# Arief-AK/OpenCL-Development-Real-time-Image-Processing

Hardware: AMD Instinct MI355X
Metric: Mpixels/s (Gaussian 5x5, 4K RGBA) (higher is better)
Workload: dtype u8 in/out, f32 accumulate

## Files before the change

### include/mi355_imgfilter.h

```cpp
#ifndef MI355_IMGFILTER_H
#define MI355_IMGFILTER_H

#include <stddef.h>
#include <stdint.h>

#ifdef __cplusplus
extern "C" {
#endif

#define MI355_OK 0
#define MI355_ERR_BAD_ARG (-1)
#define MI355_ERR_HIP (-2)
#define MI355_ERR_NO_DEVICE (-3)
#define MI355_ERR_UNSUPPORTED (-4)
#define MI355_ERR_NOMEM (-5)

#define MI355_MAX_GAUSS_K 63

#define MI355_GAUSS_FAST 0
#define MI355_GAUSS_EXACT 1

typedef struct mi355_ctx mi355_ctx;

int mi355_device_count(int* count);
// ... 15 lines not shown

#define MI355_INPUT_RGBA 0
#define MI355_INPUT_BGR 1
int mi355_ctx_set_input_format(mi355_ctx* ctx, int format);
int mi355_bgr_to_rgba8_dev(mi355_ctx* ctx, const void* d_bgr, void* d_rgba, int w, int h, int nframes);

int mi355_gauss_weights(int k, float sigma, float* out_k2);
int mi355_ctx_set_gauss_weights(mi355_ctx* ctx, int k, float sigma, const float* w_k2);

int mi355_gray_rgba8(mi355_ctx* ctx, const uint8_t* rgba, uint8_t* out_rgba, int w, int h,
                     uint64_t prof_ns[6]);
int mi355_gray1_rgba8(mi355_ctx* ctx, const uint8_t* rgba, uint8_t* out_gray, int w, int h,
                      uint64_t prof_ns[6]);
int mi355_gauss_rgba8(mi355_ctx* ctx, const uint8_t* rgba, uint8_t* out_rgba, int w, int h, int k,
                      float sigma, uint64_t prof_ns[6]);
int mi355_sobel_rgba8(mi355_ctx* ctx, const uint8_t* rgba, uint8_t* out_gray, int w, int h,
                      uint64_t prof_ns[6]);
int mi355_pipeline_rgba8(mi355_ctx* ctx, const uint8_t* rgba, uint8_t* out_gray, int w, int h, int k,
                         float sigma, uint64_t prof_ns[6]);

int mi355_image2d_rgba8(mi355_ctx* ctx, int filter, const uint8_t* rgba, uint8_t* out, int w, int h, int k,
                        float sigma, uint64_t prof_ns[6]);
int mi355_gauss_weights_image2d(int k, float sigma, float* out_k2);

#define MI355_FILTER_GRAY 0
#define MI355_FILTER_GRAY1 1
#define MI355_FILTER_GAUSS 2
#define MI355_FILTER_SOBEL 3
#define MI355_FILTER_PIPELINE 4
#define MI355_FILTER_GAUSS_GRAY8 5
#define MI355_FILTER_SOBEL_GRAY8 6
#define MI355_FILTER_PIPELINE_GRAY8 7
#define MI355_MAX_MEDIAN_K 7
#define MI355_FILTER_MEDIAN 16
#define MI355_FILTER_MEDIAN_GRAY8 17
#define MI355_MAX_MORPH_K 17
#define MI355_FILTER_ERODE 24
#define MI355_FILTER_DILATE 25
#define MI355_FILTER_OPEN 26
#define MI355_FILTER_CLOSE 27
#define MI355_FILTER_ERODE_GRAY8 28
#define MI355_FILTER_DILATE_GRAY8 29
#define MI355_FILTER_OPEN_GRAY8 30
#define MI355_FILTER_CLOSE_GRAY8 31
#define MI355_FILTER_EQUALIZE_GRAY8 40
#define MI355_FILTER_OTSU_GRAY8 41
#define MI355_MAX_BOX_K 63
#define MI355_FILTER_BOX 48
#define MI355_FILTER_BOX_GRAY8 49
int mi355_filter_batched(mi355_ctx* ctx, int filter, const uint8_t* rgba, uint8_t* out, int w, int h,
                         int nframes, int k, float sigma, uint64_t prof_ns[6]);
int mi355_filter_out_bpp(int filter);
int mi355_filter_in_bpp(int filter);

int mi355_filter_stream(mi355_ctx* ctx, int filter, const uint8_t* rgba, uint8_t* out, int w, int h,
                        int nframes, int chunk_frames, int k, float sigma, double* elapsed_ms);
int mi355_host_alloc(mi355_ctx* ctx, size_t nbytes, void** h_ptr);
int mi355_host_free(mi355_ctx* ctx, void* h_ptr);

int mi355_gray_rgba8_dev(mi355_ctx* ctx, const void* d_in, void* d_out, int w, int h, int nframes);
int mi355_gray1_rgba8_dev(mi355_ctx* ctx, const void* d_in, void* d_out, int w, int h, int nframes);
int mi355_gauss_rgba8_dev(mi355_ctx* ctx, const void* d_in, void* d_out, int w, int h, int nframes,
                          int k, float sigma);
int mi355_sobel_rgba8_dev(mi355_ctx* ctx, const void* d_in, void* d_out, int w, int h, int nframes);
int mi355_pipeline_rgba8_dev(mi355_ctx* ctx, const void* d_in, void* d_out, int w, int h, int nframes,
                             int k, float sigma);
int mi355_filter_dev(mi355_ctx* ctx, int filter, const void* d_in, void* d_out, int w, int h,
                     int nframes, int k, float sigma);
int mi355_hist_gray8_dev(mi355_ctx* ctx, const void* d_in, uint32_t* d_hist, int w, int h, int nframes);
int mi355_otsu_thresholds_gray8_dev(mi355_ctx* ctx, const void* d_in, int32_t* d_thresh, int w, int h, int nframes);

#define MI355_INTERP_NEAREST 0
#define MI355_INTERP_LINEAR 1
#define MI355_INTERP_AREA 3
#define MI355_MAX_AREA_FACTOR 16
int mi355_resize_check(int bpp, int src_w, int src_h, int dst_w, int dst_h, int nframes, int interp);
int mi355_resize_dev(mi355_ctx* ctx, const void* d_in, void* d_out, int bpp, int src_w, int src_h,
                     int dst_w, int dst_h, int nframes, int interp);
int mi355_resize_batched(mi355_ctx* ctx, const uint8_t* in, uint8_t* out, int bpp, int src_w, int src_h,
                         int dst_w, int dst_h, int nframes, int interp, uint64_t prof_ns[6]);

#define MI355_WARP_INVERSE_MAP 16
#define MI355_BORDER_CONSTANT 0
#define MI355_BORDER_REPLICATE 1
#define MI355_MAX_WARP_SIZE 32766
int mi355_rotation_matrix(double cx, double cy, double angle_deg, double scale, double m[6]);
int mi355_warp_affine_matrix(const double m[6], int flags, double inv[6]);
int mi355_warp_affine_check(int bpp, int src_w, int src_h, int dst_w, int dst_h, int nframes, const double m[6],
                            int flags, int border_mode);
int mi355_warp_affine_dev(mi355_ctx* ctx, const void* d_in, void* d_out, int bpp, int src_w, int src_h, int dst_w,
                          int dst_h, int nframes, const double m[6], int flags, int border_mode,
                          uint32_t border_value);
int mi355_warp_affine_batched(mi355_ctx* ctx, const uint8_t* in, uint8_t* out, int bpp, int src_w, int src_h,
                              int dst_w, int dst_h, int nframes, const double m[6], int flags, int border_mode,
                              uint32_t border_value, uint64_t prof_ns[6]);

#define MI355_MAP_FIXED 0
#define MI355_MAP_FLOAT 1
int mi355_remap_check(int bpp, int src_w, int src_h, int dst_w, int dst_h, int nframes, int map_kind, int interp,
                      int border_mode);
int mi355_remap_dev(mi355_ctx* ctx, const void* d_in, void* d_out, int bpp, int src_w, int src_h, int dst_w, int dst_h,
                    int nframes, const void* d_map1, const void* d_map2, int map_kind, int interp, int border_mode,
                    uint32_t border_value);
int mi355_remap_batched(mi355_ctx* ctx, const uint8_t* in, uint8_t* out, int bpp, int src_w, int src_h, int dst_w,
                        int dst_h, int nframes, const void* map1, const void* map2, int map_kind, int interp,
                        int border_mode, uint32_t border_value, uint64_t prof_ns[6]);
// ... 91 lines not shown
```

### opencl-development-real-time-image-processing_amd/__init__.py

```python
from .imgfilter import (
    ADAPTIVE_BINARY,
    ADAPTIVE_BINARY_INV,
    BORDER_CONSTANT,
    BORDER_REPLICATE,
    FILTER_BOX,
    FILTER_BOX_GRAY8,
    FILTER_CLOSE,
    FILTER_CLOSE_GRAY8,
    FILTER_DILATE,
    FILTER_DILATE_GRAY8,
    FILTER_ERODE,
    FILTER_ERODE_GRAY8,
    FILTER_EQUALIZE_GRAY8,
    FILTER_GAUSS,
    FILTER_GAUSS_GRAY8,
    FILTER_GRAY,
    FILTER_GRAY1,
    FILTER_MEDIAN,
    FILTER_MEDIAN_GRAY8,
    FILTER_OPEN,
    FILTER_OPEN_GRAY8,
    FILTER_OTSU_GRAY8,
    FILTER_PIPELINE,
    FILTER_PIPELINE_GRAY8,
    FILTER_SOBEL,
    FILTER_SOBEL_GRAY8,
    IN_BPP,
    OUT_BPP,
    GAUSS_EXACT,
    GAUSS_FAST,
    IMPL_AUTO,
    IMPL_MFMA,
    INPUT_BGR,
    INTERP_AREA,
    INTERP_LINEAR,
    INTERP_NEAREST,
    INPUT_RGBA,
    IMPL_TILE,
    IMPL_VALU,
    MAP_FIXED,
    MAP_FLOAT,
    MAX_AREA_FACTOR,
    MAX_BOX_K,
    MAX_CLAHE_TILES,
    MAX_MEDIAN_K,
    MAX_MORPH_K,
    MAX_WARP_SIZE,
    WARP_INVERSE_MAP,
    YUV_BT601,
    YUV_BT601_FULL,
    YUV_BT709,
    YUV_I420,
    YUV_NV12,
    YUV_NV21,
    YUV_UYVY,
    YUV_YUY2,
    YUV_YV12,
    Context,
    Group,
    Mi355Error,
    adaptive_threshold_check,
    build_library,
    clahe_check,
    declared_symbols,
    gauss_weights,
    gauss_weights_image2d,
    group_shard,
    library_path,
    load_library,
    perspective_matrix,
    remap_check,
    resize_check,
    rotation_matrix,
    warp_affine_check,
    warp_affine_matrix,
    warp_perspective_check,
    yuv_check,
    yuv_frame_bytes,
)
```

### opencl-development-real-time-image-processing_amd/csrc/capi.hip

```cpp
#include <hip/hip_runtime.h>

#include <cmath>
#include <cstdio>
#include <cstdlib>
#include <cstring>
#include <ctime>
#include <new>
#include <vector>

#include "../../include/mi355_imgfilter.h"
#include "kernels.hpp"

using namespace mi355;

namespace {

struct CoefEntry {
    int k;
    uint32_t sigma_bits;
    GaussCoef coef;
    float* d_buf;
    std::vector<float> h_tab;
    uint64_t last_use;
    bool installed;
// ... 853 lines not shown
}

MI355_API int mi355_gauss_weights_image2d(int k, float sigma, float* out_k2)
{
    if (!out_k2 || !valid_k(k) || !valid_sigma(sigma))
        return MI355_ERR_BAD_ARG;
    gen_weights_image2d(k, sigma, out_k2);
    return MI355_OK;
}

MI355_API int mi355_image2d_rgba8(mi355_ctx* ctx, int filter, const uint8_t* rgba, uint8_t* out, int w, int h, int k,
                                  float sigma, uint64_t prof_ns[6])
{
    if (!ctx || !rgba || !out || !valid_sizes(w, h, 1) ||
        (filter != MI355_FILTER_GRAY && filter != MI355_FILTER_GAUSS && filter != MI355_FILTER_SOBEL))
        return MI355_ERR_BAD_ARG;
    const bool gauss = filter == MI355_FILTER_GAUSS;
    if (gauss && (!valid_k(k) || !valid_sigma(sigma)))
        return MI355_ERR_BAD_ARG;
    HIP_TRY(ctx, hipSetDevice(ctx->device));
    const size_t npx = (size_t)w * h, in_bytes = npx * 4, out_bytes = npx * (gauss ? 4 : 1);
    int rc = ensure(ctx, ctx->d_in, in_bytes);
    if (rc == MI355_OK)
        rc = ensure(ctx, ctx->d_out, out_bytes);
    if (rc != MI355_OK)
        return rc;
    if (gauss) {
        if (!ctx->d_img_table)
            HIP_TRY(ctx, hipMalloc((void**)&ctx->d_img_table, sizeof(float) * MI355_MAX_GAUSS_K * MI355_MAX_GAUSS_K));
        std::vector<float> table((size_t)k * k);
        gen_weights_image2d(k, sigma, table.data());
        HIP_TRY(ctx, hipStreamSynchronize(ctx->stream));
        HIP_TRY(ctx, hipMemcpy(ctx->d_img_table, table.data(), sizeof(float) * table.size(), hipMemcpyHostToDevice));
    }
    return timed_roundtrip(ctx, ctx->d_in.p, rgba, in_bytes, out, out_bytes, prof_ns, [&] {
        HIP_TRY(ctx, launch_image2d(ctx->stream, filter, static_cast<const uint8_t*>(ctx->d_in.p),
                                    static_cast<uint8_t*>(ctx->d_out.p), w, h, 1, k, ctx->d_img_table));
        return MI355_OK;
    });
}

MI355_API int mi355_ctx_set_gauss_weights(mi355_ctx* ctx, int k, float sigma, const float* w_k2)
{
    if (!ctx || !w_k2 || !valid_k(k) || !valid_sigma(sigma))
        return MI355_ERR_BAD_ARG;
    for (int i = 0; i < k * k; i++)
        if (!std::isfinite(w_k2[i]))
            return MI355_ERR_BAD_ARG;
    HIP_TRY(ctx, hipSetDevice(ctx->device));
    HIP_TRY(ctx, hipStreamSynchronize(ctx->stream));
    return install_coef(ctx, k, sigma, w_k2, true, nullptr);
}

MI355_API int mi355_filter_out_bpp(int filter)
{
    const FilterInfo* f = filter_info(filter);
    return f ? f->out_bpp : MI355_ERR_BAD_ARG;
}

MI355_API int mi355_filter_in_bpp(int filter)
{
    const FilterInfo* f = filter_info(filter);
    return f ? f->in_bpp : MI355_ERR_BAD_ARG;
}

MI355_API int mi355_gray_rgba8(mi355_ctx* ctx, const uint8_t* rgba, uint8_t* out, int w, int h,
                               uint64_t prof_ns[6])
{
    return run_host(ctx, MI355_FILTER_GRAY, rgba, out, w, h, 1, 0, 0.0f, prof_ns);
}

MI355_API int mi355_gray1_rgba8(mi355_ctx* ctx, const uint8_t* rgba, uint8_t* out, int w, int h,
                                uint64_t prof_ns[6])
{
    return run_host(ctx, MI355_FILTER_GRAY1, rgba, out, w, h, 1, 0, 0.0f, prof_ns);
}

MI355_API int mi355_gauss_rgba8(mi355_ctx* ctx, const uint8_t* rgba, uint8_t* out, int w, int h, int k,
                                float sigma, uint64_t prof_ns[6])
{
    return run_host(ctx, MI355_FILTER_GAUSS, rgba, out, w, h, 1, k, sigma, prof_ns);
}

MI355_API int mi355_sobel_rgba8(mi355_ctx* ctx, const uint8_t* rgba, uint8_t* out, int w, int h,
                                uint64_t prof_ns[6])
{
    return run_host(ctx, MI355_FILTER_SOBEL, rgba, out, w, h, 1, 0, 0.0f, prof_ns);
}

MI355_API int mi355_pipeline_rgba8(mi355_ctx* ctx, const uint8_t* rgba, uint8_t* out, int w, int h,
                                   int k, float sigma, uint64_t prof_ns[6])
{
    return run_host(ctx, MI355_FILTER_PIPELINE, rgba, out, w, h, 1, k, sigma, prof_ns);
}

MI355_API int mi355_filter_batched(mi355_ctx* ctx, int filter, const uint8_t* rgba, uint8_t* out, int w,
                                   int h, int nframes, int k, float sigma, uint64_t prof_ns[6])
{
    return run_host(ctx, filter, rgba, out, w, h, nframes, k, sigma, prof_ns);
}

MI355_API int mi355_host_alloc(mi355_ctx* ctx, size_t nbytes, void** h_ptr)
{
    if (!ctx || !h_ptr || nbytes == 0)
        return MI355_ERR_BAD_ARG;
    HIP_TRY(ctx, hipSetDevice(ctx->device));
// ... 948 lines not shown
```

### opencl-development-real-time-image-processing_amd/csrc/gauss_slide.hip

```cpp
#include <cmath>
#include <cstdlib>
#include <type_traits>

#include "common.hpp"
#include "kernels.hpp"
#include "slide_common.hpp"

namespace mi355 {

namespace {

constexpr uint32_t kRowStoreNowhere = 0x80000000u;
__device__ __forceinline__ void gstore_row_nt(global_ptr<uint8_t> rowp, uint32_t row_bytes, uint32_t off, u32x4 v)
{
    const auto rsrc = __builtin_amdgcn_make_buffer_rsrc((void*)rowp, (short)0, (int)row_bytes, 0x00020000);
    __builtin_amdgcn_raw_buffer_store_b128(v, rsrc, (int)off, 0, 2 );
}

constexpr uint32_t kSlideLdsForFiveWaves = 160u * 1024u / 5u - 1024u;
template <typename... KArgs, typename... Args>
hipError_t launch_slide_lds(void (*kernel)(KArgs...), const BandPlan& plan, uint32_t lds_bytes, hipStream_t stream,
                            Args... args)
{
    hipLaunchKernelGGL(kernel, dim3(plan.nblocks_a + plan.nblocks_b), dim3(kSlideWavesPerBlock * 64), lds_bytes, stream,
// ... 414 lines not shown
    L.g = slide_geom<4>(it.strip, lanes_out, lane, w, 16u, 16u);
    L.y0 = it.y0;
    L.nout = it.nout;
    L.h = h;
    L.w = w;
    L.row_bytes = (size_t)w * 4;
    L.fin = uniform_ptr(in + it.frame * L.row_bytes * h);
    L.fout = uniform_ptr(out + it.frame * L.row_bytes * h);
    L.edge = RaggedEdge{false, false, false, false};
    if constexpr (RAGGED) {
        if (w >= 4)
            L.g.in_off = ragged_edge_setup(L.g.q_lane, L.g.q_load, w, &L.edge);
    }
#pragma unroll
    for (int j = 0; j < 4; j++)
        L.px_off[j] = (uint32_t)clampi(L.g.x_lane + j, 0, w - 1) * 4u;

    float wv[K];
#pragma unroll
    for (int j = 0; j < K; j++) {
        wv[j] = wts.w[j];
        asm volatile("" : "+v"(wv[j]));
    }

    const bool up = (it.band & 1) != 0;
    u32x4 q3[K];
    auto run = [&](auto amode, bool preloaded) -> int {
        constexpr int AMODE = decltype(amode)::value;
        constexpr int NCH = AMODE == 0 ? 4 : 3;
        if constexpr (R <= 3) {
            if (up)
                return gauss_slide_band<R, CLAMP, NCH, RAGGED, true, AMODE, LOCKSTEP>(L, wv, alpha_hi, alpha_tab, q3, preloaded);
        }
        return gauss_slide_band<R, CLAMP, NCH, RAGGED, false, AMODE, LOCKSTEP>(L, wv, alpha_hi, alpha_tab, q3, preloaded);
    };
    auto three_channels = [&]() -> int {
        int code = run(std::integral_constant<int, 1>{}, false);
        if (code == kBandAbortUniform || code == kBandAbortUniformFirst)
            code = run(std::integral_constant<int, 2>{}, code == kBandAbortUniformFirst);
        return code;
    };
    if constexpr (MODE == 0) {
        if (three_channels() != kBandDone)
            run(std::integral_constant<int, 0>{}, false);
    } else if constexpr (MODE == 3) {
        const int code = three_channels();
        if (lane == 0)
            flags[it.work] = code == kBandDone ? 0u : 1u;
    } else {
        run(std::integral_constant<int, 0>{}, false);
    }
}

template <int R>
bool slide_plan(int w, int h, int nframes, bool ragged, StripPlan* sp, BandPlan* plan)
{
    constexpr int K = 2 * R + 1;
    *sp = make_strip_plan(w);
    if (K == 5) {
        const bool big = (size_t)sp->nstrips * ((h + 23) / 24) * nframes >= 2800;
        const int rows = (big && !ragged) ? 15 : 24;
        return make_band_plan(h, sp->nstrips, nframes, 4, rows, rows, rows, 0.0, 12, plan);
    }
    return (K == 3)   ? make_band_plan(h, sp->nstrips, nframes, 5, 12, 12, 12, 0.0, 6, plan)
                      : make_band_plan(h, sp->nstrips, nframes, 3, 96, 270, 40, 0.1, 4 * R + 4, plan);
}

template <int R>
hipError_t launch_r(hipStream_t stream, const uint8_t* d_in, uint8_t* d_out, int w, int h, int nframes,
                    const GaussCoef& coef, uint32_t* d_flags)
{
    constexpr int K = 2 * R + 1;
    constexpr bool kSplit = R >= 3;
    StripPlan sp;
    BandPlan plan;
    const bool ragged = rows_ragged(w, d_in, 16, d_out, 16) || (size_t)w * 4 > kRowStoreNowhere;
    if (!slide_plan<R>(w, h, nframes, ragged, &sp, &plan) || (kSplit && !d_flags))
        return hipErrorInvalidValue;
    const int nstrips = sp.nstrips, lanes_out = sp.lanes_out;
    Weights<K> wts;
    for (int j = 0; j < K; j++)
        wts.w[j] = coef.h_w1d[j];
    double wsum = 0.0;
    for (int j = 0; j < K; j++)
        wsum += (double)coef.h_w1d[j];
    if (!coef.d_alpha_tab)
        return hipErrorInvalidValue;
    const uint32_t alpha_hi = coef.h_alpha_tab[255];
    const uint32_t* alpha_tab = coef.d_alpha_tab;
    const bool lockstep =
        R <= 2 && !ragged && nstrips % kSlideWavesPerBlock == 0 && plan.nwork_b == 0 && plan.nwork_a >= 8192u;
    const uint32_t lds_bytes = (R == 1 && !ragged) ? kSlideLdsForFiveWaves : 0u;
    auto launch = [&](auto kernel) {
        return launch_slide_lds(kernel, plan, lds_bytes, stream, d_in, d_out, w, h, nstrips, lanes_out, plan, wts, alpha_hi,
                                alpha_tab, d_flags);
    };
    return dispatch_bool(gauss_upper_clamp(wsum), [&](auto CL) {
        return dispatch_bool(ragged, [&](auto RG) {
            if constexpr (kSplit) {
                const hipError_t e = launch(gauss_slide_kernel<R, CL.value, RG.value, 3, false>);
                return e != hipSuccess ? e : launch(gauss_slide_kernel<R, CL.value, RG.value, 4, false>);
            } else if constexpr (RG.value) {
                return launch(gauss_slide_kernel<R, CL.value, true, 0, false>);
            } else {
                return dispatch_bool(
                    lockstep, [&](auto LS) { return launch(gauss_slide_kernel<R, CL.value, false, 0, LS.value>); });
            }
        });
    });
}

}

bool gauss_slide_supported(const uint8_t* d_in, const uint8_t* d_out, int w, int h, int k)
{
    (void)h;
    (void)w;
    if (k != 3 && k != 5 && k != 7 && k != 9)
        return false;
    return aligned_to(d_in, 4) && aligned_to(d_out, 4);
}

size_t gauss_slide_flag_items(int w, int h, int nframes, int k)
{
    StripPlan sp;
    BandPlan plan;
    const hipError_t e = dispatch_int(k, std::integer_sequence<int, 7, 9>{}, [&](auto K) {
        return slide_plan<K.value / 2>(w, h, nframes, false, &sp, &plan) ? hipSuccess : hipErrorInvalidValue;
    });
    return e == hipSuccess ? (size_t)plan.nwork_a + plan.nwork_b : 0;
}

hipError_t launch_gauss_slide(hipStream_t stream, const uint8_t* d_in, uint8_t* d_out, int w, int h,
                              int nframes, const GaussCoef& coef, uint32_t* d_flags)
{
    return dispatch_int(coef.k, std::integer_sequence<int, 3, 5, 7, 9>{}, [&](auto K) {
        return launch_r<K.value / 2>(stream, d_in, d_out, w, h, nframes, coef, d_flags);
    });
}

}
```

### opencl-development-real-time-image-processing_amd/csrc/kernels.hpp

```cpp
#pragma once
#include <hip/hip_runtime.h>
#include <stdint.h>

namespace mi355 {

struct GaussCoef {
    int k;
    const float* d_w2d;
    const float* d_w1d;
    float h_w1d[64];
    const float* h_w2d;
    bool separable;
    const uint32_t* d_alpha_tab;
    uint32_t h_alpha_tab[256];
    const uint32_t* d_alpha_cpu;
    uint32_t h_alpha_cpu[256];
};

uint32_t gauss_const_alpha(const float* w1d, int k, uint32_t a);

hipError_t launch_gray(hipStream_t stream, const uint8_t* d_in, uint8_t* d_out, int w, int h,
                       int nframes, bool one_channel);

size_t gauss_flag_items(const uint8_t* d_in, const uint8_t* d_out, int w, int h, int nframes, const GaussCoef& coef,
                        bool exact, int impl);
hipError_t launch_gauss(hipStream_t stream, const uint8_t* d_in, uint8_t* d_out, int w, int h,
                        int nframes, const GaussCoef& coef, bool exact, int impl, uint32_t* d_flags);

hipError_t launch_gauss_tile(hipStream_t stream, const uint8_t* d_in, uint8_t* d_out, int w, int h,
                             int nframes, const GaussCoef& coef, bool exact);

bool gauss_slide_supported(const uint8_t* d_in, const uint8_t* d_out, int w, int h, int k);
size_t gauss_slide_flag_items(int w, int h, int nframes, int k);
hipError_t launch_gauss_slide(hipStream_t stream, const uint8_t* d_in, uint8_t* d_out, int w, int h,
                              int nframes, const GaussCoef& coef, uint32_t* d_flags);

bool gauss_wide_supported(const uint8_t* d_in, const uint8_t* d_out, int w, int h, int k);
size_t gauss_wide_flag_items(int w, int h, int nframes, int k);
hipError_t launch_gauss_wide(hipStream_t stream, const uint8_t* d_in, uint8_t* d_out, int w, int h, int nframes,
                             const GaussCoef& coef, uint32_t* d_flags);

bool gauss_exact_supported(const uint8_t* d_in, const uint8_t* d_out, int w, int h, const GaussCoef& coef);
hipError_t launch_gauss_exact(hipStream_t stream, const uint8_t* d_in, uint8_t* d_out, int w, int h, int nframes,
                              const GaussCoef& coef);

bool gauss_mfma_reg_supported(const uint8_t* d_in, const uint8_t* d_out, int w, int h, const GaussCoef& coef);
hipError_t launch_gauss_mfma_reg(hipStream_t stream, const uint8_t* d_in, uint8_t* d_out, int w, int h, int nframes,
                                 const GaussCoef& coef);

hipError_t launch_sobel(hipStream_t stream, const uint8_t* d_in, uint8_t* d_out, int w, int h,
                        int nframes, int impl);
bool sobel_slide_supported(const uint8_t* d_in, const uint8_t* d_out, int w, int h);
hipError_t launch_sobel_slide(hipStream_t stream, const uint8_t* d_in, uint8_t* d_out, int w, int h, int nframes);

hipError_t launch_pipeline(hipStream_t stream, const uint8_t* d_in, uint8_t* d_out, int w, int h,
                           int nframes, const GaussCoef& coef, bool exact, int impl);
bool pipe_slide_supported(const uint8_t* d_in, const uint8_t* d_out, int w, int h, const GaussCoef& coef, int px);
hipError_t launch_pipe_slide(hipStream_t stream, const uint8_t* d_in, uint8_t* d_out, int w, int h, int nframes,
                             const GaussCoef& coef, int px);

hipError_t launch_gauss_gray8(hipStream_t stream, const uint8_t* d_in, uint8_t* d_out, int w, int h, int nframes,
                              const GaussCoef& coef, bool exact, int impl);
hipError_t launch_sobel_gray8(hipStream_t stream, const uint8_t* d_in, uint8_t* d_out, int w, int h, int nframes);
hipError_t launch_pipeline_gray8(hipStream_t stream, const uint8_t* d_in, uint8_t* d_out, int w, int h, int nframes,
                                 const GaussCoef& coef, int impl);

hipError_t launch_median(hipStream_t stream, const uint8_t* d_in, uint8_t* d_out, int w, int h, int nframes, int k,
                         bool gray8, int impl);

hipError_t launch_morph(hipStream_t stream, const uint8_t* d_in, uint8_t* d_out, int w, int h, int nframes, int k,
                        int op, bool gray8);

hipError_t launch_hist(hipStream_t stream, const uint8_t* d_in, uint32_t* d_hist, int w, int h, int nframes);
hipError_t launch_hist_table(hipStream_t stream, const uint32_t* d_hist, uint8_t* d_lut, int32_t* d_thresh, int w,
                             int h, int nframes, bool otsu);
hipError_t launch_lut_apply(hipStream_t stream, const uint8_t* d_in, uint8_t* d_out, const uint8_t* d_lut, int w, int h,
                            int nframes);

constexpr int kClaheMaxTiles = 16;
struct ClaheGeom {
    int w, h, tiles_x, tiles_y;
    int tw, th;
    int cl;
    float lut_scale, inv_tw, inv_th;
};
hipError_t launch_clahe_hist(hipStream_t stream, const uint8_t* d_in, uint32_t* d_hist, const ClaheGeom& g, int nframes);
hipError_t launch_clahe_table(hipStream_t stream, const uint32_t* d_hist, uint8_t* d_luts, const ClaheGeom& g,
                              int nframes);
// ... 69 lines not shown
```

### opencl-development-real-time-image-processing_amd/imgfilter.py

```python
import ctypes
import os
import re
import subprocess

import numpy as np

_HERE = os.path.dirname(os.path.abspath(__file__))
_ROOT = os.path.dirname(_HERE)
_LIB = os.path.join(_HERE, "lib", "libmi355_imgfilter.so")
_HEADER = os.path.join(_ROOT, "include", "mi355_imgfilter.h")

FILTER_GRAY, FILTER_GRAY1, FILTER_GAUSS, FILTER_SOBEL, FILTER_PIPELINE = 0, 1, 2, 3, 4
FILTER_GAUSS_GRAY8, FILTER_SOBEL_GRAY8, FILTER_PIPELINE_GRAY8 = 5, 6, 7
FILTER_MEDIAN, FILTER_MEDIAN_GRAY8 = 16, 17
MAX_MEDIAN_K = 7
FILTER_ERODE, FILTER_DILATE, FILTER_OPEN, FILTER_CLOSE = 24, 25, 26, 27
FILTER_ERODE_GRAY8, FILTER_DILATE_GRAY8, FILTER_OPEN_GRAY8, FILTER_CLOSE_GRAY8 = 28, 29, 30, 31
MAX_MORPH_K = 17
FILTER_EQUALIZE_GRAY8, FILTER_OTSU_GRAY8 = 40, 41
FILTER_BOX, FILTER_BOX_GRAY8 = 48, 49
MAX_BOX_K = 63
ADAPTIVE_BINARY, ADAPTIVE_BINARY_INV = 0, 1
MAX_CLAHE_TILES = 16
INTERP_NEAREST, INTERP_LINEAR, INTERP_AREA = 0, 1, 3
# ... 100 lines not shown
        "mi355_pipeline_rgba8_dev": [_vp, _vp, _vp, _ci, _ci, _ci, _ci, ctypes.c_float],
        "mi355_filter_dev": [_vp, _ci, _vp, _vp, _ci, _ci, _ci, _ci, ctypes.c_float],
        "mi355_hist_gray8_dev": [_vp, _vp, _vp, _ci, _ci, _ci],
        "mi355_otsu_thresholds_gray8_dev": [_vp, _vp, _vp, _ci, _ci, _ci],
        "mi355_resize_check": [_ci, _ci, _ci, _ci, _ci, _ci, _ci],
        "mi355_resize_dev": [_vp, _vp, _vp, _ci, _ci, _ci, _ci, _ci, _ci, _ci],
        "mi355_resize_batched": [_vp, _u8p, _u8p, _ci, _ci, _ci, _ci, _ci, _ci, _ci, _u64p],
        "mi355_rotation_matrix": [_cd, _cd, _cd, _cd, _f64p],
        "mi355_warp_affine_matrix": [_f64p, _ci, _f64p],
        "mi355_warp_affine_check": [_ci, _ci, _ci, _ci, _ci, _ci, _f64p, _ci, _ci],
        "mi355_warp_affine_dev": [_vp, _vp, _vp, _ci, _ci, _ci, _ci, _ci, _ci, _f64p, _ci, _ci, ctypes.c_uint32],
        "mi355_warp_affine_batched": [_vp, _u8p, _u8p, _ci, _ci, _ci, _ci, _ci, _ci, _f64p, _ci, _ci, ctypes.c_uint32,
                                      _u64p],
        "mi355_remap_check": [_ci, _ci, _ci, _ci, _ci, _ci, _ci, _ci, _ci],
        "mi355_remap_dev": [_vp, _vp, _vp, _ci, _ci, _ci, _ci, _ci, _ci, _vp, _vp, _ci, _ci, _ci, ctypes.c_uint32],
        "mi355_remap_batched": [_vp, _u8p, _u8p, _ci, _ci, _ci, _ci, _ci, _ci, _vp, _vp, _ci, _ci, _ci, ctypes.c_uint32,
                                _u64p],
        "mi355_perspective_matrix": [_f64p, _ci, _f64p],
        "mi355_warp_perspective_check": [_ci, _ci, _ci, _ci, _ci, _ci, _f64p, _ci, _ci],
        "mi355_warp_perspective_dev": [_vp, _vp, _vp, _ci, _ci, _ci, _ci, _ci, _ci, _f64p, _ci, _ci, ctypes.c_uint32],
        "mi355_warp_perspective_batched": [_vp, _u8p, _u8p, _ci, _ci, _ci, _ci, _ci, _ci, _f64p, _ci, _ci,
                                           ctypes.c_uint32, _u64p],
        "mi355_adaptive_threshold_check": [_ci, _ci, _ci, _ci, _ci, _ci, ctypes.c_double],
        "mi355_adaptive_threshold_gray8_dev": [_vp, _vp, _vp, _ci, _ci, _ci, _ci, _ci, _ci, ctypes.c_double],
        "mi355_adaptive_threshold_gray8_batched": [_vp, _u8p, _u8p, _ci, _ci, _ci, _ci, _ci, _ci, ctypes.c_double,
                                                   _u64p],
        "mi355_clahe_check": [_ci, _ci, _ci, ctypes.c_double, _ci, _ci],
        "mi355_clahe_gray8_dev": [_vp, _vp, _vp, _ci, _ci, _ci, ctypes.c_double, _ci, _ci],
        "mi355_clahe_gray8_batched": [_vp, _u8p, _u8p, _ci, _ci, _ci, ctypes.c_double, _ci, _ci, _u64p],
        "mi355_clahe_luts_gray8_dev": [_vp, _vp, _vp, _ci, _ci, _ci, ctypes.c_double, _ci, _ci],
        "mi355_yuv_check": [_ci, _ci, _ci, _ci, _ci, _ci, _ci, _ci],
        "mi355_yuv_to_rgba8_dev": [_vp, _vp, _vp, _ci, _ci, _ci, _ci, _ci, _ci, _ci],
        "mi355_rgba8_to_yuv_dev": [_vp, _vp, _vp, _ci, _ci, _ci, _ci, _ci, _ci, _ci],
        "mi355_yuv_to_gray8_dev": [_vp, _vp, _vp, _ci, _ci, _ci, _ci, _ci, _ci],
        "mi355_yuv_to_rgba8_batched": [_vp, _u8p, _u8p, _ci, _ci, _ci, _ci, _ci, _ci, _ci, _u64p],
        "mi355_rgba8_to_yuv_batched": [_vp, _u8p, _u8p, _ci, _ci, _ci, _ci, _ci, _ci, _ci, _u64p],
        "mi355_synth_rgba8_dev": [_vp, _vp, _ci, _ci, _ci, _ci, ctypes.c_uint32, _ci],
        "mi355_checksum_dev": [_vp, _vp, ctypes.c_size_t, ctypes.c_uint64, _u64p],
        "mi355_stream_copy_dev": [_vp, _vp, _vp, ctypes.c_size_t],
        "mi355_selftest": [_vp, ctypes.POINTER(ctypes.c_uint32), ctypes.POINTER(ctypes.c_uint32)],
        "mi355_dev_alloc": [_vp, ctypes.c_size_t, ctypes.POINTER(_vp)],
        "mi355_pool_alloc": [_vp, _ci, _ci, _ci, _ci, _ci, ctypes.c_float, _ci, ctypes.POINTER(_vp), ctypes.POINTER(_vp),
                             _f32p],
        "mi355_pool_free": [_vp, _vp, _vp],
        "mi355_dev_free": [_vp, _vp],
        "mi355_copy_h2d": [_vp, _vp, _vp, ctypes.c_size_t],
        "mi355_copy_d2h": [_vp, _vp, _vp, ctypes.c_size_t],
        "mi355_group_create": [_ci, ctypes.POINTER(_ci), ctypes.POINTER(_vp)],
        "mi355_group_destroy": [_vp],
        "mi355_group_size": [_vp, ctypes.POINTER(_ci)],
        "mi355_group_member_ctx": [_vp, _ci, ctypes.POINTER(_vp)],
        "mi355_group_member_status": [_vp, _ci],
        "mi355_group_shard": [_ci, _ci, _ci, ctypes.POINTER(_ci), ctypes.POINTER(_ci)],
        "mi355_group_set_gauss_mode": [_vp, _ci],
        "mi355_group_set_impl": [_vp, _ci],
        "mi355_group_set_input_format": [_vp, _ci],
        "mi355_group_set_gauss_weights": [_vp, _ci, ctypes.c_float, _f32p],
        "mi355_group_filter_batched": [_vp, _ci, _u8p, _u8p, _ci, _ci, _ci, _ci, ctypes.c_float,
                                       ctypes.POINTER(ctypes.c_double)],
        "mi355_group_filter_dev": [_vp, _ci, ctypes.POINTER(_vp), ctypes.POINTER(_vp), _ci, _ci, ctypes.POINTER(_ci), _ci,
                                   ctypes.c_float],
        "mi355_timer_begin": [_vp],
        "mi355_timer_end": [_vp, _f32p],
    }
    for name, args in sig.items():
        try:
            fn = getattr(lib, name)
        except AttributeError:
            if path == _LIB:
                raise
            continue
        fn.argtypes = args
        fn.restype = _ci
    if hasattr(lib, "mi355_yuv_frame_bytes") or path == _LIB:
        lib.mi355_yuv_frame_bytes.argtypes = [_ci, _ci, _ci, _ci, _ci]
        lib.mi355_yuv_frame_bytes.restype = ctypes.c_size_t
    lib.mi355_strerror.argtypes = [_ci]
    lib.mi355_strerror.restype = ctypes.c_char_p
    lib.mi355_build_info.argtypes = []
    lib.mi355_build_info.restype = ctypes.c_char_p
    if not other:
        _lib = lib
    return lib


def _check(fn, rc, ctx=None):
    if rc != 0:
        lib = load_library()
        detail = lib.mi355_strerror(rc).decode()
        if ctx is not None and rc == -2:
            detail += ", hipError=%d" % lib.mi355_last_hip_error(ctx)
        raise Mi355Error(fn, rc, detail)


def gauss_weights(k, sigma):
    out = np.empty((k, k), np.float32) if k > 0 else np.empty((1, 1), np.float32)
    rc = load_library().mi355_gauss_weights(int(k), float(sigma), out.ctypes.data_as(_f32p))
    _check("mi355_gauss_weights", rc)
    return out


def gauss_weights_image2d(k, sigma):
    out = np.empty((k, k), np.float32) if k > 0 else np.empty((1, 1), np.float32)
    rc = load_library().mi355_gauss_weights_image2d(int(k), float(sigma), out.ctypes.data_as(_f32p))
    _check("mi355_gauss_weights_image2d", rc)
    return out
# ... 547 lines not shown
        _check("mi355_stream_copy_dev", rc, self._h)

    def selftest(self):
        a, b = ctypes.c_uint32(0), ctypes.c_uint32(0)
        _check("mi355_selftest", self._lib.mi355_selftest(self._h, ctypes.byref(a), ctypes.byref(b)), self._h)
        return a.value, b.value

    def pool_alloc(self, filt, w, h, nframes, k=5, sigma=1.5, tries=4):
        a, b = _vp(), _vp()
        ms = (ctypes.c_float * max(1, tries))()
        rc = self._lib.mi355_pool_alloc(self._h, int(filt), int(w), int(h), int(nframes), int(k), float(sigma),
                                        int(tries), ctypes.byref(a), ctypes.byref(b), ms)
        _check("mi355_pool_alloc", rc, self._h)
        return a.value, b.value, [float(x) for x in ms][:max(1, tries)]

    def pool_free(self, d_in, d_out):
        _check("mi355_pool_free", self._lib.mi355_pool_free(self._h, _vp(int(d_in or 0)), _vp(int(d_out or 0))),
               self._h)

    def alloc(self, nbytes):
        p = _vp()
        _check("mi355_dev_alloc", self._lib.mi355_dev_alloc(self._h, int(nbytes), ctypes.byref(p)), self._h)
        return p.value

    def free(self, d_ptr):
        _check("mi355_dev_free", self._lib.mi355_dev_free(self._h, _vp(int(d_ptr))), self._h)

    def h2d(self, d_dst, arr):
        arr = np.ascontiguousarray(arr)
        rc = self._lib.mi355_copy_h2d(self._h, _vp(int(d_dst)), _vp(arr.ctypes.data), arr.nbytes)
        _check("mi355_copy_h2d", rc, self._h)

    def d2h(self, arr, d_src):
        assert arr.flags["C_CONTIGUOUS"]
        rc = self._lib.mi355_copy_d2h(self._h, _vp(arr.ctypes.data), _vp(int(d_src)), arr.nbytes)
        _check("mi355_copy_d2h", rc, self._h)

    def timer_begin(self):
        _check("mi355_timer_begin", self._lib.mi355_timer_begin(self._h), self._h)

    def timer_end(self):
        ms = ctypes.c_float(0)
        _check("mi355_timer_end", self._lib.mi355_timer_end(self._h, ctypes.byref(ms)), self._h)
        return ms.value


def group_shard(member, nmembers, nframes):
    a, b = _ci(0), _ci(0)
    _check("mi355_group_shard", load_library().mi355_group_shard(int(member), int(nmembers), int(nframes),
                                                                  ctypes.byref(a), ctypes.byref(b)))
    return a.value, b.value


class Group:

    def __init__(self, devices):
        self._lib = load_library()
        self._h = _vp()
        devs = (_ci * len(devices))(*[int(d) for d in devices])
        _check("mi355_group_create", self._lib.mi355_group_create(len(devices), devs, ctypes.byref(self._h)))
        self.size = len(devices)

    def close(self):
        if self._h:
            self._lib.mi355_group_destroy(self._h)
            self._h = _vp()

    def __enter__(self):
        return self

    def __exit__(self, *a):
        self.close()

    def __del__(self):
        try:
            self.close()
        except Exception:
            pass

    def member(self, i):
        h = _vp()
        _check("mi355_group_member_ctx", self._lib.mi355_group_member_ctx(self._h, int(i), ctypes.byref(h)))
        c = Context.__new__(Context)
        c._lib, c._h = self._lib, h
        c.close = lambda: None
        return c

    def member_status(self, i):
        return self._lib.mi355_group_member_status(self._h, int(i))

    def set_gauss_mode(self, mode):
        _check("mi355_group_set_gauss_mode", self._lib.mi355_group_set_gauss_mode(self._h, int(mode)))

    def set_impl(self, impl):
        _check("mi355_group_set_impl", self._lib.mi355_group_set_impl(self._h, int(impl)))

    def set_input_format(self, fmt):
        _check("mi355_group_set_input_format", self._lib.mi355_group_set_input_format(self._h, int(fmt)))
        self._in_ch = 3 if fmt == INPUT_BGR else 4

    def set_gauss_weights(self, k, sigma, table):
        table = np.ascontiguousarray(table, np.float32)
        rc = self._lib.mi355_group_set_gauss_weights(self._h, int(k), float(sigma), table.ctypes.data_as(_f32p))
        _check("mi355_group_set_gauss_weights", rc)

    def filter_batched(self, filt, frames, k=0, sigma=0.0, out=None):
# ... 19 lines not shown
```

Measured before the change: 771,300.

## Add small-batch Gaussian 5x5 kernel with short fixed bands for more parallel work

Result: no change. 771,000 (median of 3 runs) (-0.0%).

```diff
diff --git a/include/mi355_imgfilter.h b/include/mi355_imgfilter.h
--- a/include/mi355_imgfilter.h
+++ b/include/mi355_imgfilter.h
@@ -91,6 +91,7 @@
                          int nframes, int k, float sigma, uint64_t prof_ns[6]);
 int mi355_filter_out_bpp(int filter);
 int mi355_filter_in_bpp(int filter);
+int mi355_gauss_plan(int w, int h, int nframes, int k, int* band_rows, int* work_items, int* small_launch);
 
 int mi355_filter_stream(mi355_ctx* ctx, int filter, const uint8_t* rgba, uint8_t* out, int w, int h,
                         int nframes, int chunk_frames, int k, float sigma, double* elapsed_ms);
diff --git a/opencl-development-real-time-image-processing_amd/__init__.py b/opencl-development-real-time-image-processing_amd/__init__.py
--- a/opencl-development-real-time-image-processing_amd/__init__.py
+++ b/opencl-development-real-time-image-processing_amd/__init__.py
@@ -63,6 +63,7 @@
     build_library,
     clahe_check,
     declared_symbols,
+    gauss_plan,
     gauss_weights,
     gauss_weights_image2d,
     group_shard,
diff --git a/opencl-development-real-time-image-processing_amd/csrc/capi.hip b/opencl-development-real-time-image-processing_amd/csrc/capi.hip
--- a/opencl-development-real-time-image-processing_amd/csrc/capi.hip
+++ b/opencl-development-real-time-image-processing_amd/csrc/capi.hip
@@ -929,6 +929,17 @@
     return install_coef(ctx, k, sigma, w_k2, true, nullptr);
 }
 
+MI355_API int mi355_gauss_plan(int w, int h, int nframes, int k, int* band_rows, int* work_items, int* small_launch)
+{
+    GaussSlidePlanInfo info;
+    if (!band_rows || !work_items || !small_launch || !gauss_slide_plan_info(w, h, nframes, k, &info))
+        return MI355_ERR_BAD_ARG;
+    *band_rows = info.rows;
+    *work_items = (int)info.nwork;
+    *small_launch = info.small;
+    return MI355_OK;
+}
+
 MI355_API int mi355_filter_out_bpp(int filter)
 {
     const FilterInfo* f = filter_info(filter);
diff --git a/opencl-development-real-time-image-processing_amd/csrc/gauss_slide.hip b/opencl-development-real-time-image-processing_amd/csrc/gauss_slide.hip
--- a/opencl-development-real-time-image-processing_amd/csrc/gauss_slide.hip
+++ b/opencl-development-real-time-image-processing_amd/csrc/gauss_slide.hip
@@ -490,6 +490,189 @@
     }
 }
 
+constexpr int kSmallRows = 5;
+struct SmallPlan {
+    int rows, nbands;
+    uint32_t nwork, nblocks;
+    uint64_t inv_strips, inv_items;
+};
+constexpr uint32_t kSmallPlanMaxWork = 1u << 20;
+
+__device__ __forceinline__ uint32_t small_div(uint32_t work, uint64_t inv)
+{
+    return (uint32_t)(((uint64_t)work * inv) >> 40);
+}
+
+template <int B, bool UP>
+__device__ __forceinline__ int gauss_small_band(global_ptr<const uint8_t> fin, global_ptr<uint8_t> fout, uint32_t row_bytes,
+                                                const SlideGeom& g, int y0, int nout, int h, const Weights<5>& wts,
+                                                uint32_t alpha_hi, const uint32_t* __restrict__ alpha_tab)
+{
+    constexpr int R = 2, K = 5, NIN = B + 2 * R;
+    const BandWalk W = band_walk(UP, y0, nout, R, h);
+    const ptrdiff_t step_bytes = UP ? -(ptrdiff_t)row_bytes : (ptrdiff_t)row_bytes;
+    const int y_lo = max(y0 - R, 0), y_hi = min(y0 + nout - 1 + R, h - 1);
+    int y_in = W.y_first;
+    auto in_p = fin + (size_t)clampi(y_in, y_lo, y_hi) * row_bytes;
+    uint32_t in_off = g.in_off;
+    lane_offset_here(in_off);
+    u32x4 q[NIN];
+#pragma unroll
+    for (int i = 0; i < NIN; i++) {
+        q[i] = gload<u32x4>(in_p + in_off);
+        const int y_next = y_in + W.y_step;
+        in_p += (min(y_in, y_next) >= y_lo && max(y_in, y_next) <= y_hi) ? step_bytes : (ptrdiff_t)0;
+        y_in = y_next;
+    }
+    float wv[K];
+#pragma unroll
+    for (int j = 0; j < K; j++) {
+        wv[j] = wts.w[j];
+        asm volatile("" : "+v"(wv[j]));
+    }
+    const uint32_t out_voff = g.stores ? g.out_off : kRowStoreNowhere;
+    auto out_p = fout + (size_t)out_row(W, 0) * row_bytes;
+    float rows[K][12];
+    uint32_t cur_nA = 0u;
+    int run = 0;
+
+    auto row = [&](auto self, auto iv) __attribute__((always_inline)) -> int {
+        constexpr int I = decltype(iv)::value;
+        if constexpr (I < NIN) {
+            if (I <= 2 * R || I - 2 * R < nout) {
+                constexpr int u = I % K;
+                u32x4 p = q[I];
+                if (alpha_row_differs<false>(p, cur_nA)) {
+                    const uint32_t a_new = ((uint32_t)__builtin_amdgcn_readfirstlane((int)p.x) >> 24) & 0xFFu;
+                    const uint32_t nA = (a_new ^ 0xFFu) << 24;
+                    if (alpha_row_differs<false>(p, nA))
+                        return kBandAbort;
+                    cur_nA = nA;
+                    alpha_hi = __builtin_amdgcn_readfirstlane(alpha_tab[a_new]);
+                    run = 0;
+                }
+                run++;
+                if (g.edge_strip) {
+                    if (g.left_of_image)
+                        p = u32x4{p.x, p.x, p.x, p.x};
+                    if (g.right_of_image)
+                        p = u32x4{p.w, p.w, p.w, p.w};
+                }
+#pragma unroll
+                for (int px = 0; px < 4; px++)
+#pragma unroll
+                    for (int c = 0; c < 3; c++)
+                        rows[u][px * 3 + c] = ubyte_f32(p[px], c);
+                if constexpr (I >= 2 * R) {
+                    if (run < K)
+                        return kBandAbort;
+                    auto vsum = [&](int e) -> float {
+                        float a = wv[0] * rows[UP ? u : (u + 1) % K][e];
+#pragma unroll
+                        for (int j = 1; j < K; j++)
+                            a = __builtin_fmaf(wv[j], rows[UP ? (u - j + K) % K : (u + 1 + j) % K][e], a);
+                        return a;
+                    };
+                    float hres[4][4];
+#pragma unroll
+                    for (int c = 0; c < 3; c++)
+                        hpass5_dpp(vsum(0 * 3 + c), vsum(1 * 3 + c), vsum(2 * 3 + c), vsum(3 * 3 + c), wv[0], wv[1], wv[2],
+                                   wv[3], wv[4], hres[c][0], hres[c][1], hres[c][2], hres[c][3]);
+                    u32x4 o;
+                    cvt_pack3x4(hres, alpha_hi, o);
+                    gstore_row_nt(out_p, row_bytes, out_voff, o);
+                    out_p += step_bytes;
+                }
+                return self(self, std::integral_constant<int, I + 1>{});
+            }
+        }
+        return kBandDone;
+    };
+    return row(row, std::integral_constant<int, 0>{});
+}
+
+__global__ __launch_bounds__(kSlideWavesPerBlock * 64, 1) void gauss_small_kernel(
+    const uint8_t* __restrict__ in, uint8_t* __restrict__ out, int w, int h, int nstrips, int lanes_out, SmallPlan plan,
+    Weights<5> wts, uint32_t alpha_hi, const uint32_t* __restrict__ alpha_tab)
+{
+    constexpr int R = 2, K = 5;
+    const int lane = threadIdx.x & 63;
+    const uint32_t blk = xcd_remap(blockIdx.x, plan.nblocks);
+    const uint32_t work = __builtin_amdgcn_readfirstlane(blk * kSlideWavesPerBlock + (uint32_t)(threadIdx.x >> 6));
+    if (work >= plan.nwork)
+        return;
+    const uint32_t frame = small_div(work, plan.inv_items), in_row_of_strips = small_div(work, plan.inv_strips);
+    const int strip = (int)(work - in_row_of_strips * (uint32_t)nstrips);
+    const int band = (int)(in_row_of_strips - frame * (uint32_t)plan.nbands);
+    const int y0 = band * plan.rows, nout = min(plan.rows, h - y0);
+    const size_t row_bytes = (size_t)w * 4;
+    const SlideGeom g = slide_geom<4>(strip, lanes_out, lane, w, 16u, 16u);
+    const auto fin = uniform_ptr(in + frame * row_bytes * h);
+    const auto fout = uniform_ptr(out + frame * row_bytes * h);
+    const bool up = (band & 1) != 0;
+    constexpr int B = kSmallRows;
+    const int code = up ? gauss_small_band<B, true>(fin, fout, (uint32_t)row_bytes, g, y0, nout, h, wts, alpha_hi, alpha_tab)
+                        : gauss_small_band<B, false>(fin, fout, (uint32_t)row_bytes, g, y0, nout, h, wts, alpha_hi, alpha_tab);
+    if (code == kBandDone)
+        return;
+    SlideLane L;
+    L.g = g;
+    L.y0 = y0;
+    L.nout = nout;
+    L.h = h;
+    L.w = w;
+    L.row_bytes = row_bytes;
+    L.fin = fin;
+    L.fout = fout;
+    L.edge = RaggedEdge{false, false, false, false};
+#pragma unroll
+    for (int j = 0; j < 4; j++)
+        L.px_off[j] = 0u;
+    float wv[K];
+#pragma unroll
+    for (int j = 0; j < K; j++) {
+        wv[j] = wts.w[j];
+        asm volatile("" : "+v"(wv[j]));
+    }
+    u32x4 q3[K];
+    if (up)
+        gauss_slide_band<R, false, 4, false, true, 0, false>(L, wv, alpha_hi, alpha_tab, q3, false);
+    else
+        gauss_slide_band<R, false, 4, false, false, 0, false>(L, wv, alpha_hi, alpha_tab, q3, false);
+}
+
+constexpr size_t kSmallMaxStripRows = 2u * 16u * 2160u;
+constexpr int kSmallMaxFrames = 8;
+
+inline bool small_plan(int h, int nstrips, int nframes, SmallPlan* out)
+{
+    static const struct Tune {
+        size_t max_strip_rows = kSmallMaxStripRows;
+        Tune()
+        {
+            if (tune_env("MI355_TUNE_BAND_ROWS"))
+                max_strip_rows = 0;
+            if (const char* e = tune_env("MI355_TUNE_SMALL_MAX"))
+                max_strip_rows = (size_t)atoll(e);
+        }
+    } tune;
+    const size_t strip_rows = (size_t)nstrips * h * nframes;
+    if (strip_rows > tune.max_strip_rows || nframes > kSmallMaxFrames)
+        return false;
+    SmallPlan p{};
+    p.rows = kSmallRows;
+    p.nbands = (h + p.rows - 1) / p.rows;
+    const size_t per_frame = (size_t)nstrips * p.nbands, nwork = per_frame * nframes;
+    if (nwork == 0 || nwork > kSmallPlanMaxWork)
+        return false;
+    p.nwork = (uint32_t)nwork;
+    p.nblocks = (p.nwork + kSlideWavesPerBlock - 1) / kSlideWavesPerBlock;
+    p.inv_strips = ((1ull << 40) + (uint64_t)nstrips - 1) / (uint64_t)nstrips;
+    p.inv_items = ((1ull << 40) + per_frame - 1) / per_frame;
+    *out = p;
+    return true;
+}
+
 template <int R>
 bool slide_plan(int w, int h, int nframes, bool ragged, StripPlan* sp, BandPlan* plan)
 {
@@ -526,6 +709,17 @@
         return hipErrorInvalidValue;
     const uint32_t alpha_hi = coef.h_alpha_tab[255];
     const uint32_t* alpha_tab = coef.d_alpha_tab;
+    if constexpr (R == 2) {
+        SmallPlan small;
+        if (!ragged && !gauss_upper_clamp(wsum) && small_plan(h, nstrips, nframes, &small)) {
+            auto launch_small = [&](auto kernel) {
+                hipLaunchKernelGGL(kernel, dim3(small.nblocks), dim3(kSlideWavesPerBlock * 64), 0, stream, d_in, d_out, w, h,
+                                   nstrips, lanes_out, small, wts, alpha_hi, alpha_tab);
+                return hipGetLastError();
+            };
+            return launch_small(gauss_small_kernel);
+        }
+    }
     const bool lockstep =
         R <= 2 && !ragged && nstrips % kSlideWavesPerBlock == 0 && plan.nwork_b == 0 && plan.nwork_a >= 8192u;
     const uint32_t lds_bytes = (R == 1 && !ragged) ? kSlideLdsForFiveWaves : 0u;
@@ -569,6 +763,26 @@
     return e == hipSuccess ? (size_t)plan.nwork_a + plan.nwork_b : 0;
 }
 
+bool gauss_slide_plan_info(int w, int h, int nframes, int k, GaussSlidePlanInfo* info)
+{
+    if (w <= 0 || h <= 0 || nframes <= 0 || !info)
+        return false;
+    const hipError_t e = dispatch_int(k, std::integer_sequence<int, 3, 5, 7, 9>{}, [&](auto K) {
+        StripPlan sp;
+        BandPlan plan;
+        const bool ragged = (w & 3) != 0 || (size_t)w * 4 > kRowStoreNowhere;
+        if (!slide_plan<K.value / 2>(w, h, nframes, ragged, &sp, &plan))
+            return hipErrorInvalidValue;
+        SmallPlan small;
+        if (K.value == 5 && !ragged && small_plan(h, sp.nstrips, nframes, &small))
+            *info = GaussSlidePlanInfo{small.rows, 0, small.nwork, 1};
+        else
+            *info = GaussSlidePlanInfo{plan.rows_a, plan.nbands_b ? plan.rows_b : 0, plan.nwork_a + plan.nwork_b, 0};
+        return hipSuccess;
+    });
+    return e == hipSuccess;
+}
+
 hipError_t launch_gauss_slide(hipStream_t stream, const uint8_t* d_in, uint8_t* d_out, int w, int h,
                               int nframes, const GaussCoef& coef, uint32_t* d_flags)
 {
diff --git a/opencl-development-real-time-image-processing_amd/csrc/kernels.hpp b/opencl-development-real-time-image-processing_amd/csrc/kernels.hpp
--- a/opencl-development-real-time-image-processing_amd/csrc/kernels.hpp
+++ b/opencl-development-real-time-image-processing_amd/csrc/kernels.hpp
@@ -34,6 +34,12 @@
 size_t gauss_slide_flag_items(int w, int h, int nframes, int k);
 hipError_t launch_gauss_slide(hipStream_t stream, const uint8_t* d_in, uint8_t* d_out, int w, int h,
                               int nframes, const GaussCoef& coef, uint32_t* d_flags);
+struct GaussSlidePlanInfo {
+    int rows, rows_tail;
+    uint32_t nwork;
+    int small;
+};
+bool gauss_slide_plan_info(int w, int h, int nframes, int k, GaussSlidePlanInfo* info);
 
 bool gauss_wide_supported(const uint8_t* d_in, const uint8_t* d_out, int w, int h, int k);
 size_t gauss_wide_flag_items(int w, int h, int nframes, int k);
diff --git a/opencl-development-real-time-image-processing_amd/imgfilter.py b/opencl-development-real-time-image-processing_amd/imgfilter.py
--- a/opencl-development-real-time-image-processing_amd/imgfilter.py
+++ b/opencl-development-real-time-image-processing_amd/imgfilter.py
@@ -176,6 +176,7 @@
         "mi355_group_member_ctx": [_vp, _ci, ctypes.POINTER(_vp)],
         "mi355_group_member_status": [_vp, _ci],
         "mi355_group_shard": [_ci, _ci, _ci, ctypes.POINTER(_ci), ctypes.POINTER(_ci)],
+        "mi355_gauss_plan": [_ci, _ci, _ci, _ci, ctypes.POINTER(_ci), ctypes.POINTER(_ci), ctypes.POINTER(_ci)],
         "mi355_group_set_gauss_mode": [_vp, _ci],
         "mi355_group_set_impl": [_vp, _ci],
         "mi355_group_set_input_format": [_vp, _ci],
@@ -829,6 +830,13 @@
     return a.value, b.value
 
 
+def gauss_plan(w, h, nframes, k):
+    rows, work, small = _ci(0), _ci(0), _ci(0)
+    _check("mi355_gauss_plan", load_library().mi355_gauss_plan(int(w), int(h), int(nframes), int(k), ctypes.byref(rows),
+                                                                ctypes.byref(work), ctypes.byref(small)))
+    return rows.value, work.value, bool(small.value)
+
+
 class Group:
 
     def __init__(self, devices):
```
